# lilinitsy/skele-raytracer

Hardware: AMD Instinct MI355X
Metric: Mrays/sec + frame ms, 1920x1080 gillum=16 spheres2.scn (higher is better)
Workload: dtype f32

## Files before the change

skele_raytracer_amd/csrc/api.cpp:

```cpp
#include <hip/hip_runtime.h>

#include <cmath>
#include <cstdlib>
#include <cstdio>
#include <cstring>
#include <initializer_list>
#include <memory>
#include <vector>

#include "launch.h"
#include "scene_host.h"

static thread_local const char *g_variant = "none";

#define SKR_HIP(call)                                                                                      \
	do                                                                                                     \
	{                                                                                                      \
		hipError_t e_ = (call);                                                                            \
		if(e_ != hipSuccess)                                                                               \
		{                                                                                                  \
			skr_set_error("%s failed: %s (%s:%d)", #call, hipGetErrorString(e_), __FILE__, __LINE__);     \
			return SKR_ERR_HIP;                                                                            \
		}                                                                                                  \
	} while(0)
// ... 2 lines not shown
	int device = 0;
	skr_scene_info info{};
	int lds_limit = 0;
	int pow_steps = 11;
	float4 *d_blob = nullptr;
	size_t blob_bytes = 0;
	float4 *d_camec = nullptr;
	unsigned long long *d_counters = nullptr;
	unsigned long long *d_tri_work = nullptr;
	size_t off_amb = 0, off_kd = 0, off_ks = 0, off_lights = 0, off_tris = 0, off_chunks = 0, off_tri_mats = 0;
	size_t off_fog = 0;
	int n_fog = 0;
	size_t off_spot = 0;
	int n_spot = 0, spot_first = 0;
	size_t off_smask = 0;
	float shadow_reach2 = 0.0f;
	size_t off_gi = 0;
	SkrGiGrid gi_grid[2] = {};
	uint32_t gi_mask_word = 0;
	int gi_wide = 0;
	size_t gi_surface_word = 0;
	int n_chunks = 0, chunk_size = 0, cones = 0;
	size_t chunk_stride = 0;
	size_t off_trace = 0;
	float4 trace_ball{};
	int trace_cones = 0;
	bool tri_shadows = false;
	bool sphere_tree = false;
	size_t off_st_rows = 0, off_st_chunks = 0, off_st_nodes = 0;
	int st_nodes = 0, st_chunks = 0, st_always = 0;
// ... 63 lines not shown
	const int rc = r->nodes.grow(need);
	if(kept) *kept = rc == SKR_OK && was_kept && r->nodes.bytes == had;
	return rc;
}

static void load_switches(SkrSwitches &sw)
{
	sw = SkrSwitches();
	if(const char *e = getenv("SKR_PIPELINE"))
		sw.pipeline = !strcmp(e, "nodes") ? SKR_PIPE_NODES : !strcmp(e, "generic") ? SKR_PIPE_GENERIC : SKR_PIPE_OTHER;
	sw.no_cones = getenv("SKR_NO_CONES") != nullptr;
	sw.no_cull = getenv("SKR_NO_CULL") != nullptr;
	if(const char *e = getenv("SKR_NO_SPHERE_CULL")) sw.no_sphere_cull = atoi(e) > 0 ? 1 : 0;
	if(const char *e = getenv("SKR_LEVELS_BUDGET_MB")) sw.budget_mb = atoi(e) > 0 ? atoi(e) : 1;
	if(const char *e = getenv("SKR_FLAT")) sw.flat = atoi(e) > 0 ? 1 : -1;
	if(const char *e = getenv("SKR_SHADOW_MASK")) sw.shadow_mask = atoi(e) > 0 ? 1 : 0;
	if(const char *e = getenv("SKR_GI_MASK")) sw.gi_mask = atoi(e) > 0 ? 1 : 0;
	if(const char *e = getenv("SKR_GI_SURFACE")) sw.gi_surface = atoi(e) > 0 ? 1 : 0;
	if(const char *e = getenv("SKR_PRIMARY_CACHE")) sw.primary_cache = atoi(e) > 0 ? 1 : 0;
	if(const char *e = getenv("SKR_ADAPTIVE_PATH")) sw.adaptive_path = !strcmp(e, "frame") ? 1 : !strcmp(e, "query") ? 2 : 0;
}

void skr_copy_switches(skr_renderer *dst, const skr_renderer *src) { dst->sw = src->sw; }
int skr_render_tile_list_owned(skr_renderer *r, const skr_options *opt, uint32_t tile_rows, const uint32_t *d_tiles, uint32_t n_slots, uint64_t table_id, uint8_t *d_rgb,
							   float *d_rgbf, void *stream);

static std::vector<skr_f4> pack_scene(const skr_scene &s, DeviceScene &d)
{
	std::vector<skr_f4> rows;
	auto put = [&](const void *src, size_t bytes) {
		const size_t at = rows.size();
		rows.resize(at + (bytes + 15) / 16, skr_f4{0.0f, 0.0f, 0.0f, 0.0f});
		if(src && bytes) memcpy(&rows[at], src, bytes);
// ... 13 lines not shown
	d.n_chunks = s.info.n_triangles ? s.tri_node_count : 0;
	d.off_tri_mats = put4(s.tri_mats);
	d.off_fog = rows.size();
	d.n_fog = (int) (s.raw_fog.size() / 9);
	for(int j = 0; j < d.n_fog; j++)
	{
		const float *f = &s.raw_fog[9 * j];
		rows.push_back({f[3], f[8], f[7], 0.0f});
		rows.push_back({f[4], f[5], f[6], 0.0f});
	}
	d.n_spot = s.n_spot();
	d.spot_first = s.info.n_point_lights;
	d.off_spot = put4(s.spot_cones);
	if(!s.shadow_masks.empty()) d.off_smask = put(s.shadow_masks.data(), s.shadow_masks.size() * 4);
	d.shadow_reach2 = s.shadow_reach2;
	if(!s.gi_table.empty())
	{
		const size_t patch_word = s.gi_mask_word + (size_t) s.gi_rows * (SKR_GI_ROW_ENTRIES * (s.gi_wide ? 4 : 2) / 4);
		d.gi_surface_word = s.gi_surface.empty() ? 0 : patch_word + s.gi_surface_head;
		d.off_gi = put(nullptr, std::max(s.gi_table.size(), s.gi_surface.empty() ? 0 : patch_word + s.gi_surface.size()) * 4);
		uint32_t *words = reinterpret_cast<uint32_t *>(&rows[d.off_gi]);
		memcpy(words, s.gi_table.data(), s.gi_table.size() * 4);
		if(d.gi_surface_word) memcpy(words + patch_word, s.gi_surface.data(), s.gi_surface.size() * 4);
	}
	d.gi_grid[0] = s.gi_grid[0];
	d.gi_grid[1] = s.gi_grid[1];
	d.gi_mask_word = s.gi_mask_word;
	d.gi_wide = s.gi_wide;
	if(s.info.n_triangles && !s.trace_chunks.empty()) d.off_trace = put4(s.trace_chunks);
	d.trace_ball = make_float4(s.trace_ball[0], s.trace_ball[1], s.trace_ball[2], s.trace_ball[3]);
// ... 238 lines not shown
	const float *c = s.info.camera;
	p.background = f3{s.info.background[0], s.info.background[1], s.info.background[2]};
	p.n_spheres = s.info.n_spheres;
	p.n_tris = s.info.n_triangles;
	p.n_lights = s.info.n_point_lights + s.n_spot + s.info.n_directional_lights;
	p.sph_geom = s.d_blob;
	p.cam_ec = s.d_camec;
	p.sph_amb = s.d_blob + s.off_amb;
	p.sph_kd = s.d_blob + s.off_kd;
	p.sph_ks = s.d_blob + s.off_ks;
	p.lights = s.d_blob + s.off_lights;
	p.tris = s.d_blob + s.off_tris;
	p.tri_chunks = s.d_blob + s.off_chunks;
	p.tri_chunk_size = s.chunk_size;
	p.tri_cones = (s.cones && !r->sw.no_cones) ? 1 : 0;
	if(s.off_smask && r->sw.shadow_mask)
	{
		p.shadow_masks = reinterpret_cast<const uint32_t *>(s.d_blob + s.off_smask);
		p.shadow_reach2 = s.shadow_reach2;
		p.shadow_all = p.n_spheres >= 32 ? ~0u : (1u << p.n_spheres) - 1u;
	}
	if(s.off_gi && r->sw.gi_mask)
	{
		p.gi_index = reinterpret_cast<const int32_t *>(s.d_blob + s.off_gi);
		p.gi_masks = reinterpret_cast<const uint32_t *>(s.d_blob + s.off_gi) + s.gi_mask_word;
		p.gi_grid[0] = s.gi_grid[0];
		p.gi_grid[1] = s.gi_grid[1];
		p.gi_wide = s.gi_wide;
		p.gi_all = p.n_spheres >= 32 ? ~0u : (1u << p.n_spheres) - 1u;
		if(s.gi_surface_word && r->sw.gi_surface) p.gi_surface = reinterpret_cast<const uint32_t *>(s.d_blob + s.off_gi) + s.gi_surface_word;
	}
	{
		auto len3 = [](const float *v) { return std::sqrt((double) v[0] * v[0] + (double) v[1] * v[1] + (double) v[2] * v[2]); };
		const double umax = std::fabs((double) p.angle * p.aspect) * 1.001, vmax = std::fabs((double) p.angle) * 1.001;
		const double dmax = len3(c + 3) + umax * len3(c + 9) + vmax * len3(c + 6);
// ... 884 lines not shown
```

skele_raytracer_amd/csrc/render_params.h:

```cpp
#pragma once

#include <hip/hip_runtime.h>
#include <stdint.h>

#include "shadow_cells.h"

struct f3 {
	float x, y, z;
};

#define SKR_COUNTER_SHARDS 4096u
#ifndef SKR_PULL_QUEUES
#define SKR_PULL_QUEUES 16u
#endif
#define SKR_PULL_STRIDE 256u
#define SKR_P1_REGIONS 64u
#define SKR_PREFIX_WORDS (SKR_P1_REGIONS + 1u)

enum SkrPipeline { SKR_PIPE_AUTO = 0, SKR_PIPE_NODES, SKR_PIPE_GENERIC, SKR_PIPE_OTHER };
struct SkrSwitches {
	int32_t pipeline = SKR_PIPE_AUTO;
	int8_t no_cones = 0, no_cull = 0;
	int8_t primary_cache = 1;
	int8_t no_sphere_cull = 0;
	int32_t budget_mb = 0;
	int32_t flat = 0;
	int8_t shadow_mask = 1;
	int8_t gi_mask = 1;
	int8_t gi_surface = 1;
	int8_t adaptive_path = 0;
};

static_assert(sizeof(SkrSwitches) == 20, "SkrSwitches keeps its 20 bytes");

struct RenderParams {
	SkrSwitches sw;
	int32_t width, height;
	uint32_t tile_rows, first_tile, tile_stride, out_rows;
	const uint32_t *tile_table;
	uint32_t band_row0, band_rows;
	float inv_width, inv_height, aspect, angle;
	f3 cam_pos, cam_dir, cam_up, cam_right, background;
	int32_t n_spheres, n_tris, n_lights;
	const float4 *sph_geom, *sph_amb, *sph_kd, *sph_ks, *lights, *tris;
	const float4 *cam_ec;
	const float4 *tri_chunks;
	int32_t tri_chunk_size;
	int32_t tri_cones;
	int32_t n_tri_chunks;
	int32_t monte_carlo, num_path_traces, grid_size, max_depth, use_shadows;
	uint32_t seed_lo, seed_hi;
	int32_t pow_steps;
	uint8_t *rgb;
	float *rgbf;
	unsigned long long *counters;
	unsigned long long *tri_work;
	uint32_t *qctr;
	float *acc;
	uint32_t aa_index;
	uint32_t fog_row;
	const float4 *nd_src;
	const float4 *ns_src;
	float4 *nd_dst, *ns_dst;
	uint32_t nd_src_level0;
	const uint32_t *nd_count;
	float4 *rc;
	uint32_t rc_cap;
	uint32_t *rc_ctr;
	uint4 *ixh;
	uint32_t band_blk0, band_nblk, blocks_x;
	void *node_scratch;
	const float *res_in;
	float *res_out;
	int32_t shade_triangles;
	int32_t legacy_reflect;
	const float4 *tri_mats;
	uint32_t g_level;
	uint32_t g_arity;
	uint32_t g_last;
// ... 1 lines not shown
	const float4 *g_nodes_src;
	union {
		float4 *g_nodes_dst;
		int32_t *gi_row0;
	};
	const uint32_t *shadow_masks;
	float shadow_reach2;
	uint32_t shadow_all;
	const int32_t *gi_index;
	const uint32_t *gi_masks;
	SkrGiGrid gi_grid[2];
	int32_t gi_wide;
	uint32_t gi_all;
	const uint32_t *gi_surface;
};

struct SphereTree {
	const float4 *nodes;
	const float4 *chunks;
	const float4 *rows;
	int32_t n_nodes;
	int32_t n_chunks;
	int32_t n_always;
	int32_t cull;
	float4 ball;
	unsigned long long *work;
};

struct SpotLights {
	const float4 *cones;
// ... 21 lines not shown
```

skele_raytracer_amd/csrc/scene_host.cpp:

```cpp
#include "scene_host.h"

#include <cstdarg>
#include <cstdio>
#include <cstdlib>
#include <cstring>
#include <algorithm>
#include <cmath>
#include <fstream>

static thread_local char g_err[512] = "";

void skr_set_error(const char *fmt, ...)
{
	va_list ap;
	va_start(ap, fmt);
	vsnprintf(g_err, sizeof g_err, fmt, ap);
	va_end(ap);
}

extern "C" const char *skr_last_error(void) { return g_err; }

namespace {

int read_floats(const char *p, float *dst, int n)
// ... 79 lines not shown
	{
		const float *t = &raw_triangles[(size_t) order[i] * 9];
		tris[3 * i] = {t[0], t[1], t[2], 0.0f};
		float file_index;
		const int32_t fi = order[i];
		memcpy(&file_index, &fi, 4);
		tris[3 * i + 1] = {t[3] - t[0], t[4] - t[1], t[5] - t[2], file_index};
		tris[3 * i + 2] = {t[6] - t[0], t[7] - t[1], t[8] - t[2], 0.0f};
	}
	tri_order = order;
	build_triangle_materials();
	build_triangle_chunks();
	build_shadow_masks();
	build_gi_masks();
	build_gi_surface();
}

void skr_scene::build_lights()
{
	const int nl = info.n_point_lights, nsp = n_spot();
	const int nd = (int) (raw_directional_lights.size() / 6);
	lights.resize((size_t) (nl + nsp + nd) * 2);
	for(int i = 0; i < nl; i++)
	{
		const float *l = &raw_point_lights[(size_t) i * 6];
		lights[2 * i] = {l[0], l[1], l[2], 0.0f};
		lights[2 * i + 1] = {l[3], l[4], l[5], 0.0f};
	}
	spot_cones.resize((size_t) nsp * 2);
	for(int i = 0; i < nsp; i++)
// ... 126 lines not shown
			const double S = qn + rk;
			const double base = rk + eps_o + eta * (S + D + eps_o) / (1.0 - eta) + 0x1p-30 * qn;
			for(int c = 0; c < SKR_SHADOW_TABLE_WORDS; c++)
			{
				const double *wc = &cell_dir[3 * (size_t) c];
				const double s = q[0] * wc[0] + q[1] * wc[1] + q[2] * wc[2];
				const double dist = std::sqrt(std::max(0.0, qq - s * s));
				if(dist <= base + cell_theta[c] * S) masks[(size_t) l * SKR_SHADOW_TABLE_WORDS + c] |= 1u << k;
			}
		}
	}
	shadow_masks.swap(masks);
	shadow_reach2 = reach2;
}

static void gi_ball_bits(const double *q, double rho, const double *C, double r2, uint32_t bit, const std::vector<double> &cell_dir,
						 const std::vector<double> &cth, const std::vector<double> &sth, uint32_t *row)
{
	const double v[3] = {C[0] - q[0], C[1] - q[1], C[2] - q[2]};
	const double dist = std::sqrt(v[0] * v[0] + v[1] * v[1] + v[2] * v[2]);
	const double E = (dist + rho) * (1.0 + 0x1p-20);
	const double rk = std::sqrt(r2 + 0x1p-16 * (E * E + r2)) + 0x1p-20 * E;
	const double tol = 0x1p-30 * (dist + rho + rk);
	const double behind = rho + 0x1p-16 * E + tol;
	const double reach = rk + rho + tol;
	if(dist <= reach)
	{
		for(int e = 0; e < SKR_GI_ROW_ENTRIES; e++) row[e] |= bit;
		return;
	}
	for(int e = 0; e < SKR_GI_ROW_ENTRIES; e++)
	{
		const double *w = &cell_dir[3 * (size_t) e];
		const double cp = (v[0] * w[0] + v[1] * w[1] + v[2] * w[2]) / dist;
		const double x = v[1] * w[2] - v[2] * w[1], y = v[2] * w[0] - v[0] * w[2], z = v[0] * w[1] - v[1] * w[0];
		const double sp = std::sqrt(x * x + y * y + z * z) / dist;
		const double ct = cth[e], st = sth[e];
		const bool lo0 = cp >= ct;
		const bool hipi = cp <= -ct;
		const double cos_lo = lo0 ? 1.0 : cp * ct + sp * st;
		const double sin_lo = lo0 ? 0.0 : sp * ct - cp * st;
		const double sin_hi = hipi ? 0.0 : sp * ct + cp * st;
		const double min_sin = std::max(0.0, std::min(sin_lo, sin_hi));
		if(dist * cos_lo + behind >= 0.0 && dist * min_sin <= reach) row[e] |= bit;
	}
}

void skr_scene::build_gi_masks()
{
	gi_table.clear();
	gi_grid[0] = gi_grid[1] = SkrGiGrid{};
	gi_mask_word = 0;
	gi_wide = 0;
	const int ns = info.n_spheres;
	if(ns < 1 || ns > SKR_GI_MAX_SPHERES || info.n_triangles > 0) return;
	std::vector<double> C((size_t) 3 * ns), r2(ns), rad(ns);
	for(int k = 0; k < ns; k++)
	{
		C[3 * k] = sph_geom[k].x;
		C[3 * k + 1] = sph_geom[k].y;
// ... 107 lines not shown
	}
	std::vector<uint32_t> masks(cells.size() * SKR_GI_ROW_ENTRIES, 0u);
	for(size_t ci = 0; ci < cells.size(); ci++)
		for(int k = 0; k < ns; k++) gi_ball_bits(cells[ci].q, cells[ci].rho, &C[3 * k], r2[k], 1u << k, cell_dir, cth, sth, &masks[ci * SKR_GI_ROW_ENTRIES]);
	const size_t n_index = (index.size() + 1) & ~(size_t) 1;
	const size_t n_mask_words = gi_wide ? masks.size() : masks.size() / 2;
	std::vector<uint32_t> table((n_index + n_mask_words + 3) & ~(size_t) 3, 0u);
	memcpy(table.data(), index.data(), index.size() * 4);
	if(gi_wide) memcpy(&table[n_index], masks.data(), masks.size() * 4);
	else
		for(size_t e = 0; e < masks.size(); e += 2) table[n_index + e / 2] = masks[e] | masks[e + 1] << 16;
	gi_mask_word = (uint32_t) n_index;
	gi_table.swap(table);
}

void skr_scene::build_gi_surface()
{
	gi_surface.clear();
	gi_surface_head = 0;
	gi_rows = 0;
	if(gi_table.empty()) return;
	const int ns = info.n_spheres;
	const size_t row_words = (size_t) SKR_GI_ROW_ENTRIES * (gi_wide ? 4 : 2) / 4;
	gi_rows = (uint32_t) ((gi_table.size() - gi_mask_word) / row_words);
	std::vector<double> C((size_t) 3 * ns), r2(ns), rad(ns), R_lo(ns), R_hi(ns);
	std::vector<float> tau(ns);
	for(int k = 0; k < ns; k++)
	{
		C[3 * k] = sph_geom[k].x;
		C[3 * k + 1] = sph_geom[k].y;
		C[3 * k + 2] = sph_geom[k].z;
		r2[k] = sph_geom[k].w;
		rad[k] = std::sqrt(r2[k]);
		tau[k] = rad[k] > 1e-3 ? (float) (r2[k] * 0x1p-7) : -1.0f;
		R_lo[k] = std::sqrt(std::max(0.0, (r2[k] - tau[k]) * (1.0 - 0x1p-20))) * (1.0 - 0x1p-22);
		R_hi[k] = std::sqrt((r2[k] + std::max(0.0f, tau[k])) * (1.0 + 0x1p-20)) * (1.0 + 0x1p-22);
	}
	double blo[3], bhi[3];
	for(int c = 0; c < 3; c++)
	{
		blo[c] = gi_grid[0].lo[c];
		bhi[c] = blo[c] + gi_grid[0].n[c] / (double) gi_grid[0].inv;
	}
	struct Patch {
		int s, cell;
		double q[3], rho;
	};
	std::vector<Patch> patches;
	std::vector<int> G(ns, 0);
	std::vector<std::vector<double>> cdir(ns), cth(ns);
	size_t n_index = 0;
	bool fits = false;
	std::vector<double> sorted(rad);
	std::sort(sorted.begin(), sorted.end());
	double small_area = 0.0;
	for(int k = 0; k < ns; k++)
		if(rad[k] <= 4.0 * sorted[ns / 2]) small_area += 24.0 * r2[k];
	double edge = std::max(1e-6, 0.5 * std::sqrt(small_area / std::max(1.0, (double) SKR_GI_MAX_BYTES / (row_words * 4))));
	for(int attempt = 0; attempt < 200 && !fits; attempt++, edge *= 1.15)
	{
		patches.clear();
		n_index = 0;
		for(int k = 0; k < ns; k++)
		{
			const int g = tau[k] < 0.0f ? 0 : (int) std::min((double) SKR_GI_SURFACE_MAX_CELLS, std::max(1.0, std::ceil(2.0 * rad[k] / edge)));
			if(g != G[k])
			{
				G[k] = g;
				cdir[k].clear();
				cth[k].clear();
				if(g) cube_cells(g, cdir[k], cth[k]);
				for(double &t : cth[k]) t = t * (1.0 + 0x1p-20) + 0x1p-20;
			}
			n_index += (size_t) 6 * g * g;
			for(int cell = 0; cell < 6 * g * g; cell++)
			{
				const double *w = &cdir[k][3 * (size_t) cell];
				const double th = cth[k][cell], h = rad[k] * std::cos(th);
				Patch pt;
				pt.s = k;
				pt.cell = cell;
				for(int c = 0; c < 3; c++) pt.q[c] = C[3 * k + c] + h * w[c];
				double far = 0.0;
				for(double R : {R_lo[k], R_hi[k]}) far = std::max(far, std::sqrt(std::max(0.0, R * R + h * h - 2.0 * R * h * std::cos(th))));
				double cmax = 0.0;
				for(int c = 0; c < 3; c++) cmax = std::max(cmax, std::fabs(C[3 * k + c]));
				pt.rho = far * (1.0 + 0x1p-20) + 0x1p-30 * (cmax + rad[k]);
				double gap2 = 0.0;
				for(int c = 0; c < 3; c++)
				{
					const double o = std::max(0.0, std::max(blo[c] - pt.q[c], pt.q[c] - bhi[c]));
					gap2 += o * o;
				}
				if(gap2 <= pt.rho * pt.rho) patches.push_back(pt);
			}
		}
		fits = (SKR_GI_SURFACE_HEAD * (size_t) ns + n_index) * 4 + patches.size() * row_words * 4 <= SKR_GI_MAX_BYTES;
	}
	if(!fits || patches.empty()) return;
	std::vector<double> cell_dir, cell_theta;
	cube_cells(SKR_GI_DIR_CELLS, cell_dir, cell_theta);
	std::vector<double> dth(SKR_GI_ROW_ENTRIES), dct(SKR_GI_ROW_ENTRIES), dst(SKR_GI_ROW_ENTRIES);
	for(int e = 0; e < SKR_GI_ROW_ENTRIES; e++)
	{
		dth[e] = cell_theta[e] * (1.0 + 0x1p-20) + 0x1p-40;
		dct[e] = std::cos(dth[e]);
		dst[e] = std::sin(dth[e]);
	}
	std::vector<uint32_t> masks(patches.size() * SKR_GI_ROW_ENTRIES, 0u);
	for(size_t pi = 0; pi < patches.size(); pi++)
	{
		const Patch &pt = patches[pi];
		uint32_t *row = &masks[pi * SKR_GI_ROW_ENTRIES];
		for(int k = 0; k < ns; k++)
// ... 19 lines not shown
	int32_t *index = reinterpret_cast<int32_t *>(head + SKR_GI_SURFACE_HEAD * ns);
	size_t at = SKR_GI_SURFACE_HEAD * (size_t) ns;
	for(int k = 0; k < ns; k++)
	{
		head[SKR_GI_SURFACE_HEAD * k] = (uint32_t) at;
		head[SKR_GI_SURFACE_HEAD * k + 1] = (uint32_t) G[k];
		const float t = G[k] ? tau[k] : -1.0f;
		memcpy(&head[SKR_GI_SURFACE_HEAD * k + 2], &t, 4);
		for(int c = 0; c < 6 * G[k] * G[k]; c++) head[at + c] = 0xffffffffu;
		at += (size_t) 6 * G[k] * G[k];
	}
	for(size_t pi = 0; pi < patches.size(); pi++)
		index[head[SKR_GI_SURFACE_HEAD * patches[pi].s] - SKR_GI_SURFACE_HEAD * ns + patches[pi].cell] = (int32_t) (gi_rows + pi);
	gi_surface_head = (uint32_t) n_mask_words;
	gi_surface.swap(table);
}

void skr_scene::build_triangle_chunks()
{
	tri_chunks.clear();
	tri_any_cone = false;
	if(info.n_triangles == 0) return;
	const double dmax[SKR_CULL_LEVELS] = SKR_CULL_DMAX_LIST;
	for(int level = 0; level < SKR_CULL_LEVELS; level++)
	{
		std::vector<skr_f4> one;
		build_triangle_chunk_level(dmax[level], one);
		tri_chunk_stride = one.size();
		tri_chunks.insert(tri_chunks.end(), one.begin(), one.end());
	}
// ... 808 lines not shown
{
	if(!scene || n < 0 || n > SKR_SPOT_MAX_LIGHTS || (n && !rows))
	{
		skr_set_error("skr_scene_set_spot_lights: bad argument (at most %d spot lights)", SKR_SPOT_MAX_LIGHTS);
		return SKR_ERR_ARG;
	}
	for(int32_t i = 0; i < n; i++)
		if(!skr_spot_row_ok(rows + (size_t) i * 11))
		{
			skr_set_error("skr_scene_set_spot_lights: row %d is not a spot light (11 finite numbers, a direction other than zero, 0 <= angle1 <= angle2 <= 180)", i);
			return SKR_ERR_ARG;
		}
	scene->raw_spot_lights.assign(rows, rows + (size_t) n * 11);
	scene->build_lights();
	scene->build_shadow_masks();
	return SKR_OK;
}

int skr_scene_get_spot_lights(const skr_scene *scene, float *rows, int32_t *n)
{
	if(!scene) return SKR_ERR_ARG;
	if(n) *n = (int32_t) scene->n_spot();
	if(rows && !scene->raw_spot_lights.empty()) memcpy(rows, scene->raw_spot_lights.data(), scene->raw_spot_lights.size() * 4);
	return SKR_OK;
}

int skr_scene_get_spot_cones(const skr_scene *scene, float *cones)
{
	if(!scene) return SKR_ERR_ARG;
	for(int i = 0; cones && i < scene->n_spot(); i++)
// ... 162 lines not shown
			const SkrGiGrid &G = scene->gi_grid[g];
			const float row[8] = {G.lo[0], G.lo[1], G.lo[2], G.inv, (float) G.n[0], (float) G.n[1], (float) G.n[2], (float) G.base};
			memcpy(grids + 8 * g, row, sizeof(row));
		}
	if(table && !scene->gi_table.empty()) memcpy(table, scene->gi_table.data(), scene->gi_table.size() * 4);
	return SKR_OK;
}

int skr_scene_get_gi_surface(const skr_scene *scene, int32_t *n_words, int32_t *head_word, int32_t *first_row, uint32_t *table)
{
	if(!scene) return SKR_ERR_ARG;
	if(n_words) *n_words = (int32_t) scene->gi_surface.size();
	if(head_word) *head_word = (int32_t) scene->gi_surface_head;
	if(first_row) *first_row = (int32_t) scene->gi_rows;
	if(table && !scene->gi_surface.empty()) memcpy(table, scene->gi_surface.data(), scene->gi_surface.size() * 4);
	return SKR_OK;
}

void skr_options_default(skr_options *opt)
{
	if(!opt) return;
	opt->width = 1920;
	opt->height = 1080;
	opt->fov = 60;
	opt->monte_carlo = 0;
	opt->num_path_traces = 1;
	opt->grid_size = 0;
	opt->max_depth = 3;
	opt->use_shadows = 0;
	opt->seed = 1;
// ... 130 lines not shown
```

skele_raytracer_amd/csrc/scene_host.h:

```cpp
#pragma once

#include <cstdint>
#include <string>
#include <vector>

#include "../../include/skr.h"
#include "shadow_cells.h"
#include "tri_chunks.h"


struct skr_f4 {
	float x, y, z, w;
};

struct skr_scene {
	std::vector<float> raw_spheres;
	std::vector<float> raw_sphere_ior;
	std::vector<float> raw_triangles;
	std::vector<float> raw_triangle_materials;
	std::vector<float> raw_point_lights;
	std::vector<float> raw_directional_lights;
	std::vector<float> raw_fog;
	std::vector<float> raw_spot_lights;
	bool strict = false;
// ... 24 lines not shown
	void build_triangle_chunk_level(double d_max, std::vector<skr_f4> &out, const double *origin_ball = nullptr);
	std::vector<skr_f4> trace_chunks;
	float trace_ball[4] = {0.0f, 0.0f, 0.0f, 0.0f};
	bool trace_any_cone = false;
	std::vector<uint32_t> shadow_masks;
	float shadow_reach2 = 0.0f;
	void build_shadow_masks();
	std::vector<uint32_t> gi_table;
	SkrGiGrid gi_grid[2] = {};
	uint32_t gi_mask_word = 0;
	int gi_wide = 0;
	void build_gi_masks();
	std::vector<uint32_t> gi_surface;
	uint32_t gi_surface_head = 0;
	uint32_t gi_rows = 0;
	void build_gi_surface();
};

#define SKR_SPHERE_CHUNK 4
#define SKR_SPHERE_SUPER 8
struct SkrSphereTree {
	int n_nodes = 0, n_chunks = 0, n_always = 0;
	std::vector<skr_f4> rows;
	std::vector<int32_t> file;
	std::vector<skr_f4> nodes;
	std::vector<skr_f4> chunks;
	float ball[4] = {0.0f, 0.0f, 0.0f, -1.0f};
};
void skr_build_sphere_tree(const skr_scene &scene, SkrSphereTree &out);

bool skr_spot_row_ok(const float row[11]);
// ... 5 lines not shown
```

skele_raytracer_amd/csrc/shade_common.h:

```cpp
#pragma once

#include "device_math.h"
#include "render_params.h"
#include "shadow_cells.h"
#include "tri_chunks.h"

namespace {


struct SceneView {
	const float4 *geom;
	const float4 *amb;
	const float4 *kd;
	const float4 *ks;
	const float4 *lights;
	const float4 *tris;
	int ns, nt, nl;
	const float4 *chunks;
	int nchunks;
	int chunk;
	int cones;
	unsigned long long *tri_work;
	const float4 *geom_u;
	const uint32_t *smask;
// ... 355 lines not shown
	occ1 = !second;
	auto test = [&](const float4 g, int i) { pair_any_step(rp, pa, o, g, i, occ0, occ1, tests); };
	if(COHERENT) table_rows<SKR_COHERENT_TRIP>(sv.geom_u, sv.ns, test, [&] { return !__all(occ0 && occ1); });
	else if(sv.smask)
	{
		diag_mask_gate(19, cand, sv.ns);
		masked_rows(sv, cand, test);
	}
	else sphere_rows(sv, test);
	if(!occ0) tests += (uint32_t) sv.ns;
	if(second && !occ1) tests += (uint32_t) sv.ns;
	if(!second) occ1 = false;
}

template <bool COHERENT>
SKR_DEV uint32_t shadow_cands(const SceneView &sv, const RenderParams &p, int i, bool second, f3 P)
{
	if(COHERENT || !sv.smask || !p.use_shadows) return 0u;
	const uint32_t m0 = shadow_mask_of(sv, i, ld3(sv.lights[2 * i]) - P);
	return second ? m0 | shadow_mask_of(sv, i + 1, ld3(sv.lights[2 * i + 2]) - P) : m0;
}

SKR_DEV bool sphere_entry_touched(f3 o, f3 d, float dd, float4 A, float kappa)
{
	const f3 e = ld3(A) - o;
	const f3 cr = cross3(e, d);
	return !(dot3(cr, cr) > (A.w + kappa * dot3(e, e)) * dd);
}

SKR_DEV void sphere_work_add(const SphereTree &st, uint32_t n_cull, uint32_t n_sph)
{
	if(st.work && (n_cull | n_sph))
	{
// ... 193 lines not shown
	t.L = to_l * lt.inv;
	t.intensity = lt.inv2;
	return t;
}

struct NoTriangleShadows {
	static constexpr bool on = false;
};

struct SphereLoopShadows {
	static constexpr bool loops = true;
};

template <bool COHERENT, typename TS = NoTriangleShadows, typename SS = SphereLoopShadows>
SKR_DEV f3 direct_light_of(const SceneView &sv, const RenderParams &p, f3 kd, f3 ks, float4 ambp, f3 P, f3 N, Counters &cn, const TS &tri_shadows = TS(),
						   const SS &sphere_shadows = SS())
{
	f3 diffuse = mk3(0, 0, 0), specular = mk3(0, 0, 0);
	const f3 view = normalize3(p.cam_pos - P);
	for(int i = 0; i < sv.nl; i += 2)
	{
		const bool second = i + 1 < sv.nl;
		const uint32_t cand = SS::loops ? shadow_cands<COHERENT>(sv, p, i, second, P) : 0u;
		const LightTerm t0 = light_term(sv, i, P), t1 = light_term(sv, second ? i + 1 : i, P);
		bool occ0 = false, occ1 = false;
		if(p.use_shadows)
		{
			cn.shadow_rays += second ? 2u : 1u;
			if constexpr(SS::loops) occluded_pair<COHERENT>(sv, P, t0.L, t1.L, second, occ0, occ1, cn.shadow_tests, cand);
			else sphere_shadows.pair(sv, P, t0.L, t1.L, second, occ0, occ1, cn.shadow_tests);
			if constexpr(TS::on) tri_shadows(P, i, second, t0.L, t1.L, occ0, occ1);
		}
		auto add_light = [&](const LightTerm &t, bool lit)
		{
			if(lit)
			{
				diffuse = diffuse + ((kd * t.lc) * t.intensity) * max0(dot3(N, t.L));
				const f3 vl = view + t.L;
// ... 77 lines not shown
			}
		};
		add_light(t0, !occ0);
		add_light(t1, !occ1);
	}
	f3 total = mk3(0, 0, 0);
	total = total + ld3(ambp);
	total = total + diffuse;
	total = total + specular;
	return total;
}

template <bool COHERENT>
SKR_DEV f3 direct_light(const SceneView &sv, const RenderParams &p, int sph, f3 P, f3 N, Counters &cn)
{
	return direct_light_of<COHERENT>(sv, p, ld3(sv.kd[sph]), ld3(sv.ks[sph]), sv.amb[sph], P, N, cn);
}

SKR_DEV f3 fog_term(float4 a, float4 alb, const LightTerm &t, f3 centre, f3 lpos, f3 kd, f3 N, const uint32_t ctr[4], uint32_t k0, uint32_t k1,
					float *no_interaction_out = nullptr)
{
	float distance = length3(centre - lpos);
	if(distance > 2 * a.x) distance = 2 * a.x;
	const float no_interaction = (float) exp_spec((double) ((-1.0f * distance) * (a.y + a.z)));
	if(no_interaction_out) *no_interaction_out = no_interaction;
	uint32_t rnd[4];
	philox4x32(ctr[0], ctr[1], ctr[2], ctr[3], k0, k1, rnd);
	if(u31_to_unit(rnd[0]) > no_interaction) return ((kd * t.lc) * t.intensity) * max0(dot3(N, t.L));
	const f3 nd = mk3(t.L.x + u31_to_pm1(rnd[1]) * a.z, t.L.y + u31_to_pm1(rnd[2]) * a.z, t.L.z + u31_to_pm1(rnd[3]) * a.z);
	return (ld3(alb) * t.lc) * max0(dot3(N, nd));
}
// ... 335 lines not shown
```

skele_raytracer_amd/csrc/shadow_cells.h:

```cpp
#pragma once

#include <stdint.h>

#ifndef SKR_SHADOW_CELLS
#define SKR_SHADOW_CELLS 32
#endif
#define SKR_SHADOW_TABLE_WORDS (6 * SKR_SHADOW_CELLS * SKR_SHADOW_CELLS)
#define SKR_SHADOW_MAX_SPHERES 32

#ifndef SKR_GI_DIR_CELLS
#define SKR_GI_DIR_CELLS 16
#endif
#define SKR_GI_ROW_ENTRIES (6 * SKR_GI_DIR_CELLS * SKR_GI_DIR_CELLS)
#define SKR_GI_MAX_SPHERES 32
#define SKR_GI_MAX_BYTES (2u << 20)
struct SkrGiGrid {
	float lo[3], inv;
	float n_f[3];
	int32_t n[3], base;
};

#define SKR_GI_SURFACE_HEAD 4
#define SKR_GI_SURFACE_MAX_CELLS 128
```

Baseline: 62710.

## Add per-surface-patch precomputed shadow candidate masks for sphere hit points

Builds a host-side table that, for each light pair and each cube-mapped patch on every sphere's surface, conservatively lists which spheres could occlude the light. When a shading point lies on its sphere's surface, the kernel reads this tighter mask instead of the per-light direction-cell masks, so fewer sphere shadow tests run. It costs more scene-build time, up to 1 MB of extra table memory, and an extra head word packed into kd.w, and it relies on the conservative bounds being correct. It is enabled by default through the shadow_mask switch bit.

```diff
diff --git a/skele_raytracer_amd/csrc/api.cpp b/skele_raytracer_amd/csrc/api.cpp
--- a/skele_raytracer_amd/csrc/api.cpp
+++ b/skele_raytracer_amd/csrc/api.cpp
@@ -40,6 +40,8 @@
 	size_t off_spot = 0;
 	int n_spot = 0, spot_first = 0;
 	size_t off_smask = 0;
+	size_t off_ssurf = 0;
+	uint32_t ssurf_stride = 0;
 	float shadow_reach2 = 0.0f;
 	size_t off_gi = 0;
 	SkrGiGrid gi_grid[2] = {};
@@ -133,9 +135,10 @@
 	if(const char *e = getenv("SKR_NO_SPHERE_CULL")) sw.no_sphere_cull = atoi(e) > 0 ? 1 : 0;
 	if(const char *e = getenv("SKR_LEVELS_BUDGET_MB")) sw.budget_mb = atoi(e) > 0 ? atoi(e) : 1;
 	if(const char *e = getenv("SKR_FLAT")) sw.flat = atoi(e) > 0 ? 1 : -1;
-	if(const char *e = getenv("SKR_SHADOW_MASK")) sw.shadow_mask = atoi(e) > 0 ? 1 : 0;
+	if(const char *e = getenv("SKR_SHADOW_MASK")) sw.shadow_mask = (sw.shadow_mask & ~1) | (atoi(e) > 0 ? 1 : 0);
 	if(const char *e = getenv("SKR_GI_MASK")) sw.gi_mask = atoi(e) > 0 ? 1 : 0;
 	if(const char *e = getenv("SKR_GI_SURFACE")) sw.gi_surface = atoi(e) > 0 ? 1 : 0;
+	if(const char *e = getenv("SKR_SHADOW_SURFACE")) sw.shadow_mask = (sw.shadow_mask & ~2) | (atoi(e) > 0 ? 2 : 0);
 	if(const char *e = getenv("SKR_PRIMARY_CACHE")) sw.primary_cache = atoi(e) > 0 ? 1 : 0;
 	if(const char *e = getenv("SKR_ADAPTIVE_PATH")) sw.adaptive_path = !strcmp(e, "frame") ? 1 : !strcmp(e, "query") ? 2 : 0;
 }
@@ -179,6 +182,12 @@
 	d.off_spot = put4(s.spot_cones);
 	if(!s.shadow_masks.empty()) d.off_smask = put(s.shadow_masks.data(), s.shadow_masks.size() * 4);
 	d.shadow_reach2 = s.shadow_reach2;
+	if(!s.shadow_surface.empty())
+	{
+		d.off_ssurf = put(s.shadow_surface.data(), s.shadow_surface.size() * 4);
+		d.ssurf_stride = s.shadow_surface_stride;
+		for(size_t k = 0; k < s.shadow_surface_head.size(); k++) memcpy(&rows[d.off_kd + k].w, &s.shadow_surface_head[k], 4);
+	}
 	if(!s.gi_table.empty())
 	{
 		const size_t patch_word = s.gi_mask_word + (size_t) s.gi_rows * (SKR_GI_ROW_ENTRIES * (s.gi_wide ? 4 : 2) / 4);
@@ -447,11 +456,16 @@
 	p.tri_chunks = s.d_blob + s.off_chunks;
 	p.tri_chunk_size = s.chunk_size;
 	p.tri_cones = (s.cones && !r->sw.no_cones) ? 1 : 0;
-	if(s.off_smask && r->sw.shadow_mask)
+	if(s.off_smask && (r->sw.shadow_mask & 1))
 	{
 		p.shadow_masks = reinterpret_cast<const uint32_t *>(s.d_blob + s.off_smask);
 		p.shadow_reach2 = s.shadow_reach2;
 		p.shadow_all = p.n_spheres >= 32 ? ~0u : (1u << p.n_spheres) - 1u;
+		if(s.off_ssurf && (r->sw.shadow_mask & 2))
+		{
+			p.shadow_surface_word = (uint32_t) ((s.off_ssurf - s.off_smask) * 4);
+			p.shadow_surface_stride = s.ssurf_stride;
+		}
 	}
 	if(s.off_gi && r->sw.gi_mask)
 	{
diff --git a/skele_raytracer_amd/csrc/render_params.h b/skele_raytracer_amd/csrc/render_params.h
--- a/skele_raytracer_amd/csrc/render_params.h
+++ b/skele_raytracer_amd/csrc/render_params.h
@@ -25,7 +25,7 @@
 	int8_t no_sphere_cull = 0;
 	int32_t budget_mb = 0;
 	int32_t flat = 0;
-	int8_t shadow_mask = 1;
+	int8_t shadow_mask = 3;
 	int8_t gi_mask = 1;
 	int8_t gi_surface = 1;
 	int8_t adaptive_path = 0;
@@ -51,6 +51,7 @@
 	int32_t monte_carlo, num_path_traces, grid_size, max_depth, use_shadows;
 	uint32_t seed_lo, seed_hi;
 	int32_t pow_steps;
+	uint32_t shadow_surface_word;
 	uint8_t *rgb;
 	float *rgbf;
 	unsigned long long *counters;
@@ -63,6 +64,7 @@
 	const float4 *ns_src;
 	float4 *nd_dst, *ns_dst;
 	uint32_t nd_src_level0;
+	uint32_t shadow_surface_stride;
 	const uint32_t *nd_count;
 	float4 *rc;
 	uint32_t rc_cap;
@@ -94,6 +96,7 @@
 	uint32_t gi_all;
 	const uint32_t *gi_surface;
 };
+static_assert(sizeof(RenderParams) == 624, "RenderParams keeps its size: new fields go into its alignment holes");
 
 struct SphereTree {
 	const float4 *nodes;
diff --git a/skele_raytracer_amd/csrc/scene_host.cpp b/skele_raytracer_amd/csrc/scene_host.cpp
--- a/skele_raytracer_amd/csrc/scene_host.cpp
+++ b/skele_raytracer_amd/csrc/scene_host.cpp
@@ -117,6 +117,7 @@
 	build_shadow_masks();
 	build_gi_masks();
 	build_gi_surface();
+	build_shadow_surface();
 }
 
 void skr_scene::build_lights()
@@ -273,36 +274,53 @@
 	shadow_reach2 = reach2;
 }
 
+struct BallSphere {
+	double v[3], dist;
+	double rk;
+	double behind, reach;
+	bool meets;
+};
+static BallSphere ball_sphere(const double *q, double rho, const double *C, double r2)
+{
+	BallSphere b;
+	for(int c = 0; c < 3; c++) b.v[c] = C[c] - q[c];
+	b.dist = std::sqrt(b.v[0] * b.v[0] + b.v[1] * b.v[1] + b.v[2] * b.v[2]);
+	const double E = (b.dist + rho) * (1.0 + 0x1p-20);
+	b.rk = std::sqrt(r2 + 0x1p-16 * (E * E + r2)) + 0x1p-20 * E;
+	const double tol = 0x1p-30 * (b.dist + rho + b.rk);
+	b.behind = rho + 0x1p-16 * E + tol;
+	b.reach = b.rk + rho + tol;
+	b.meets = b.dist <= b.reach;
+	return b;
+}
+struct ConeSphere {
+	double cos_lo, min_sin;
+};
+static ConeSphere cone_sphere(const double *v, double dist, const double *w, double ct, double st)
+{
+	const double cp = (v[0] * w[0] + v[1] * w[1] + v[2] * w[2]) / dist;
+	const double x = v[1] * w[2] - v[2] * w[1], y = v[2] * w[0] - v[0] * w[2], z = v[0] * w[1] - v[1] * w[0];
+	const double sp = std::sqrt(x * x + y * y + z * z) / dist;
+	const bool lo0 = cp >= ct;
+	const bool hipi = cp <= -ct;
+	const double sin_lo = lo0 ? 0.0 : sp * ct - cp * st;
+	const double sin_hi = hipi ? 0.0 : sp * ct + cp * st;
+	return ConeSphere{lo0 ? 1.0 : cp * ct + sp * st, std::max(0.0, std::min(sin_lo, sin_hi))};
+}
+static bool cone_ahead(const ConeSphere &c, double dist, double behind) { return dist * c.cos_lo + behind >= 0.0; }
+static bool cone_line_touches(const ConeSphere &c, double dist, double reach) { return dist * c.min_sin <= reach; }
+static bool ball_cone_touches(const BallSphere &b, const double *w, double ct, double st)
+{
+	if(b.meets) return true;
+	const ConeSphere c = cone_sphere(b.v, b.dist, w, ct, st);
+	return cone_ahead(c, b.dist, b.behind) && cone_line_touches(c, b.dist, b.reach);
+}
 static void gi_ball_bits(const double *q, double rho, const double *C, double r2, uint32_t bit, const std::vector<double> &cell_dir,
 						 const std::vector<double> &cth, const std::vector<double> &sth, uint32_t *row)
 {
-	const double v[3] = {C[0] - q[0], C[1] - q[1], C[2] - q[2]};
-	const double dist = std::sqrt(v[0] * v[0] + v[1] * v[1] + v[2] * v[2]);
-	const double E = (dist + rho) * (1.0 + 0x1p-20);
-	const double rk = std::sqrt(r2 + 0x1p-16 * (E * E + r2)) + 0x1p-20 * E;
-	const double tol = 0x1p-30 * (dist + rho + rk);
-	const double behind = rho + 0x1p-16 * E + tol;
-	const double reach = rk + rho + tol;
-	if(dist <= reach)
-	{
-		for(int e = 0; e < SKR_GI_ROW_ENTRIES; e++) row[e] |= bit;
-		return;
-	}
+	const BallSphere b = ball_sphere(q, rho, C, r2);
 	for(int e = 0; e < SKR_GI_ROW_ENTRIES; e++)
-	{
-		const double *w = &cell_dir[3 * (size_t) e];
-		const double cp = (v[0] * w[0] + v[1] * w[1] + v[2] * w[2]) / dist;
-		const double x = v[1] * w[2] - v[2] * w[1], y = v[2] * w[0] - v[0] * w[2], z = v[0] * w[1] - v[1] * w[0];
-		const double sp = std::sqrt(x * x + y * y + z * z) / dist;
-		const double ct = cth[e], st = sth[e];
-		const bool lo0 = cp >= ct;
-		const bool hipi = cp <= -ct;
-		const double cos_lo = lo0 ? 1.0 : cp * ct + sp * st;
-		const double sin_lo = lo0 ? 0.0 : sp * ct - cp * st;
-		const double sin_hi = hipi ? 0.0 : sp * ct + cp * st;
-		const double min_sin = std::max(0.0, std::min(sin_lo, sin_hi));
-		if(dist * cos_lo + behind >= 0.0 && dist * min_sin <= reach) row[e] |= bit;
-	}
+		if(ball_cone_touches(b, &cell_dir[3 * (size_t) e], cth[e], sth[e])) row[e] |= bit;
 }
 
 void skr_scene::build_gi_masks()
@@ -440,17 +458,59 @@
 	gi_table.swap(table);
 }
 
+struct SurfaceShell {
+	float tau;
+	double R_lo, R_hi;
+};
+static SurfaceShell surface_shell(double r2)
+{
+	SurfaceShell sh;
+	sh.tau = std::sqrt(r2) > 1e-3 ? (float) (r2 * 0x1p-7) : -1.0f;
+	sh.R_lo = std::sqrt(std::max(0.0, (r2 - sh.tau) * (1.0 - 0x1p-20))) * (1.0 - 0x1p-22);
+	sh.R_hi = std::sqrt((r2 + std::max(0.0f, sh.tau)) * (1.0 + 0x1p-20)) * (1.0 + 0x1p-22);
+	return sh;
+}
+static void surface_patch_ball(const double *C, double rad, const SurfaceShell &sh, const double *w, double th, double *q, double &rho)
+{
+	const double h = rad * std::cos(th);
+	for(int c = 0; c < 3; c++) q[c] = C[c] + h * w[c];
+	double far = 0.0;
+	for(double R : {sh.R_lo, sh.R_hi}) far = std::max(far, std::sqrt(std::max(0.0, R * R + h * h - 2.0 * R * h * std::cos(th))));
+	double cmax = 0.0;
+	for(int c = 0; c < 3; c++) cmax = std::max(cmax, std::fabs(C[c]));
+	rho = far * (1.0 + 0x1p-20) + 0x1p-30 * (cmax + rad);
+}
+static void surface_cells(int g, std::vector<double> &dir, std::vector<double> &theta)
+{
+	dir.clear();
+	theta.clear();
+	if(g) cube_cells(g, dir, theta);
+	for(double &t : theta) t = t * (1.0 + 0x1p-20) + 0x1p-20;
+}
+static double surface_first_edge(const std::vector<double> &rad, const std::vector<double> &r2, double rows)
+{
+	const int ns = (int) rad.size();
+	std::vector<double> sorted(rad);
+	std::sort(sorted.begin(), sorted.end());
+	double small_area = 0.0;
+	for(int k = 0; k < ns; k++)
+		if(rad[k] <= 4.0 * sorted[ns / 2]) small_area += 24.0 * r2[k];
+	return std::max(1e-6, 0.5 * std::sqrt(small_area / std::max(1.0, rows)));
+}
+
 void skr_scene::build_gi_surface()
 {
 	gi_surface.clear();
 	gi_surface_head = 0;
 	gi_rows = 0;
+	gi_surface_edge = 0.0;
 	if(gi_table.empty()) return;
 	const int ns = info.n_spheres;
 	const size_t row_words = (size_t) SKR_GI_ROW_ENTRIES * (gi_wide ? 4 : 2) / 4;
 	gi_rows = (uint32_t) ((gi_table.size() - gi_mask_word) / row_words);
 	std::vector<double> C((size_t) 3 * ns), r2(ns), rad(ns), R_lo(ns), R_hi(ns);
 	std::vector<float> tau(ns);
+	std::vector<SurfaceShell> shell(ns);
 	for(int k = 0; k < ns; k++)
 	{
 		C[3 * k] = sph_geom[k].x;
@@ -458,9 +518,10 @@
 		C[3 * k + 2] = sph_geom[k].z;
 		r2[k] = sph_geom[k].w;
 		rad[k] = std::sqrt(r2[k]);
-		tau[k] = rad[k] > 1e-3 ? (float) (r2[k] * 0x1p-7) : -1.0f;
-		R_lo[k] = std::sqrt(std::max(0.0, (r2[k] - tau[k]) * (1.0 - 0x1p-20))) * (1.0 - 0x1p-22);
-		R_hi[k] = std::sqrt((r2[k] + std::max(0.0f, tau[k])) * (1.0 + 0x1p-20)) * (1.0 + 0x1p-22);
+		shell[k] = surface_shell(r2[k]);
+		tau[k] = shell[k].tau;
+		R_lo[k] = shell[k].R_lo;
+		R_hi[k] = shell[k].R_hi;
 	}
 	double blo[3], bhi[3];
 	for(int c = 0; c < 3; c++)
@@ -477,12 +538,7 @@
 	std::vector<std::vector<double>> cdir(ns), cth(ns);
 	size_t n_index = 0;
 	bool fits = false;
-	std::vector<double> sorted(rad);
-	std::sort(sorted.begin(), sorted.end());
-	double small_area = 0.0;
-	for(int k = 0; k < ns; k++)
-		if(rad[k] <= 4.0 * sorted[ns / 2]) small_area += 24.0 * r2[k];
-	double edge = std::max(1e-6, 0.5 * std::sqrt(small_area / std::max(1.0, (double) SKR_GI_MAX_BYTES / (row_words * 4))));
+	double edge = surface_first_edge(rad, r2, (double) SKR_GI_MAX_BYTES / (row_words * 4)), used_edge = 0.0;
 	for(int attempt = 0; attempt < 200 && !fits; attempt++, edge *= 1.15)
 	{
 		patches.clear();
@@ -493,25 +549,15 @@
 			if(g != G[k])
 			{
 				G[k] = g;
-				cdir[k].clear();
-				cth[k].clear();
-				if(g) cube_cells(g, cdir[k], cth[k]);
-				for(double &t : cth[k]) t = t * (1.0 + 0x1p-20) + 0x1p-20;
+				surface_cells(g, cdir[k], cth[k]);
 			}
 			n_index += (size_t) 6 * g * g;
 			for(int cell = 0; cell < 6 * g * g; cell++)
 			{
-				const double *w = &cdir[k][3 * (size_t) cell];
-				const double th = cth[k][cell], h = rad[k] * std::cos(th);
 				Patch pt;
 				pt.s = k;
 				pt.cell = cell;
-				for(int c = 0; c < 3; c++) pt.q[c] = C[3 * k + c] + h * w[c];
-				double far = 0.0;
-				for(double R : {R_lo[k], R_hi[k]}) far = std::max(far, std::sqrt(std::max(0.0, R * R + h * h - 2.0 * R * h * std::cos(th))));
-				double cmax = 0.0;
-				for(int c = 0; c < 3; c++) cmax = std::max(cmax, std::fabs(C[3 * k + c]));
-				pt.rho = far * (1.0 + 0x1p-20) + 0x1p-30 * (cmax + rad[k]);
+				surface_patch_ball(&C[3 * k], rad[k], shell[k], &cdir[k][3 * (size_t) cell], cth[k][cell], pt.q, pt.rho);
 				double gap2 = 0.0;
 				for(int c = 0; c < 3; c++)
 				{
@@ -522,8 +568,10 @@
 			}
 		}
 		fits = (SKR_GI_SURFACE_HEAD * (size_t) ns + n_index) * 4 + patches.size() * row_words * 4 <= SKR_GI_MAX_BYTES;
+		if(fits) used_edge = edge;
 	}
 	if(!fits || patches.empty()) return;
+	gi_surface_edge = used_edge;
 	std::vector<double> cell_dir, cell_theta;
 	cube_cells(SKR_GI_DIR_CELLS, cell_dir, cell_theta);
 	std::vector<double> dth(SKR_GI_ROW_ENTRIES), dct(SKR_GI_ROW_ENTRIES), dst(SKR_GI_ROW_ENTRIES);
@@ -573,6 +621,107 @@
 		index[head[SKR_GI_SURFACE_HEAD * patches[pi].s] - SKR_GI_SURFACE_HEAD * ns + patches[pi].cell] = (int32_t) (gi_rows + pi);
 	gi_surface_head = (uint32_t) n_mask_words;
 	gi_surface.swap(table);
+}
+
+void skr_scene::build_shadow_surface(double rho_scale, double cone_scale)
+{
+	shadow_surface.clear();
+	shadow_surface_head.clear();
+	shadow_surface_stride = 0;
+	if(shadow_masks.empty()) return;
+	const int ns = info.n_spheres, nl = (int) (shadow_masks.size() / SKR_SHADOW_TABLE_WORDS), npairs = (nl + 1) / 2;
+	std::vector<double> C((size_t) 3 * ns), r2(ns), rad(ns);
+	std::vector<SurfaceShell> shell(ns);
+	for(int k = 0; k < ns; k++)
+	{
+		C[3 * k] = sph_geom[k].x;
+		C[3 * k + 1] = sph_geom[k].y;
+		C[3 * k + 2] = sph_geom[k].z;
+		r2[k] = sph_geom[k].w;
+		rad[k] = std::sqrt(r2[k]);
+		for(int c = 0; c < 3; c++)
+			if(!(std::fabs(C[3 * k + c]) < 1e6)) return;
+		if(!(rad[k] < 1e6)) return;
+		shell[k] = surface_shell(r2[k]);
+	}
+	double edge = gi_surface_edge > 0.0 ? gi_surface_edge : surface_first_edge(rad, r2, (double) SKR_GI_MAX_BYTES / (SKR_GI_ROW_ENTRIES * (ns > 16 ? 4 : 2)));
+	edge /= SKR_SHADOW_SURFACE_SCALE;
+	std::vector<int> G(ns, 0);
+	size_t stride = 0;
+	for(int attempt = 0; attempt < 200; attempt++, edge *= 1.15)
+	{
+		stride = 0;
+		for(int k = 0; k < ns; k++)
+		{
+			G[k] = shell[k].tau < 0.0f ? 0 : (int) std::min((double) SKR_GI_SURFACE_MAX_CELLS, std::max(1.0, std::ceil(2.0 * rad[k] / edge)));
+			stride += (size_t) 6 * G[k] * G[k];
+		}
+		if(stride * npairs * 4 <= SKR_SHADOW_SURFACE_MAX_BYTES) break;
+	}
+	if(stride == 0 || stride * npairs * 4 > SKR_SHADOW_SURFACE_MAX_BYTES) return;
+	const uint32_t all = ns >= 32 ? 0xffffffffu : (1u << ns) - 1u;
+	const double eta = 0x1p-15;
+	std::vector<uint32_t> table(stride * npairs, 0u), head(ns, 0u);
+	std::vector<double> cdir, cth;
+	std::vector<BallSphere> bs(ns);
+	size_t base = 0;
+	for(int s = 0; s < ns; s++)
+	{
+		head[s] = (uint32_t) base | (uint32_t) G[s] << 24;
+		surface_cells(G[s], cdir, cth);
+		double cmax = 0.0;
+		for(int c = 0; c < 3; c++) cmax = std::max(cmax, std::fabs(C[3 * s + c]));
+		const double eps_o = 2.0 * std::sqrt(3.0) * (1e-6 + 0x1p-23 * (cmax + shell[s].R_hi + 1e-6));
+		const double R_in = shell[s].R_lo - eps_o;
+		const double E_own = (shell[s].R_hi + eps_o) * (1.0 + 0x1p-20);
+		const double behind_own = 0x1p-16 * E_own + 0x1p-30 * shell[s].R_hi;
+		const double tilt = R_in > 0.0 ? std::asin(std::min(1.0, eps_o / shell[s].R_lo)) : 0.0;
+		for(int cell = 0; cell < 6 * G[s] * G[s]; cell++)
+		{
+			const double *wp = &cdir[3 * (size_t) cell];
+			double q[3], rho;
+			surface_patch_ball(&C[3 * s], rad[s], shell[s], wp, cth[cell], q, rho);
+			rho = (rho + eps_o) * rho_scale;
+			for(int k = 0; k < ns; k++)
+				if(k != s) bs[k] = ball_sphere(q, rho, &C[3 * k], r2[k]);
+			for(int l = 0; l < nl; l++)
+			{
+				uint32_t &word = table[(size_t) (l >> 1) * stride + base + cell];
+				const skr_f4 &lp = lights[2 * (size_t) l];
+				const double d[3] = {lp.x - q[0], lp.y - q[1], lp.z - q[2]};
+				const double dl = std::sqrt(d[0] * d[0] + d[1] * d[1] + d[2] * d[2]);
+				if(!(dl > rho * (1.0 + 0x1p-20) + 0x1p-30 * (cmax + rad[s])))
+				{
+					word = all;
+					continue;
+				}
+				const double w[3] = {d[0] / dl, d[1] / dl, d[2] / dl};
+				const double theta = (std::asin(std::min(1.0, rho / dl)) * (1.0 + 0x1p-20) + eta) * cone_scale;
+				const double ct = std::cos(theta), st = std::sin(theta);
+				const double near_l = eps_o + eta * (dl + rho) * (1.0 + 0x1p-20);
+				const double lpd[3] = {lp.x, lp.y, lp.z};
+				for(int k = 0; k < ns; k++)
+				{
+					if(k == s) continue;
+					const BallSphere &b = bs[k];
+					const bool ahead = b.meets || cone_ahead(cone_sphere(b.v, b.dist, w, ct, st), b.dist, b.behind);
+					const double vl[3] = {C[3 * k] - lpd[0], C[3 * k + 1] - lpd[1], C[3 * k + 2] - lpd[2]};
+					const double distl = std::sqrt(vl[0] * vl[0] + vl[1] * vl[1] + vl[2] * vl[2]);
+					const double reach_l = b.rk + near_l + 0x1p-30 * (distl + dl + b.rk);
+					const bool line = distl <= reach_l || cone_line_touches(cone_sphere(vl, distl, w, ct, st), distl, reach_l);
+					if(ahead && line) word |= 1u << k;
+				}
+				const double x = wp[1] * w[2] - wp[2] * w[1], y = wp[2] * w[0] - wp[0] * w[2], z = wp[0] * w[1] - wp[1] * w[0];
+				const double psi = std::atan2(std::sqrt(x * x + y * y + z * z), wp[0] * w[0] + wp[1] * w[1] + wp[2] * w[2]);
+				const double ang = psi + cth[cell] + tilt + theta + 0x1p-30;
+				if(!(R_in > 0.0 && ang < 0.5 * M_PI && R_in * std::cos(ang) > behind_own)) word |= 1u << s;
+			}
+		}
+		base += (size_t) 6 * G[s] * G[s];
+	}
+	shadow_surface_stride = (uint32_t) stride;
+	shadow_surface.swap(table);
+	shadow_surface_head.swap(head);
 }
 
 void skr_scene::build_triangle_chunks()
@@ -1411,6 +1560,7 @@
 	scene->raw_spot_lights.assign(rows, rows + (size_t) n * 11);
 	scene->build_lights();
 	scene->build_shadow_masks();
+	scene->build_shadow_surface();
 	return SKR_OK;
 }
 
@@ -1603,6 +1753,23 @@
 	if(head_word) *head_word = (int32_t) scene->gi_surface_head;
 	if(first_row) *first_row = (int32_t) scene->gi_rows;
 	if(table && !scene->gi_surface.empty()) memcpy(table, scene->gi_surface.data(), scene->gi_surface.size() * 4);
+	return SKR_OK;
+}
+
+int skr_scene_get_shadow_surface(const skr_scene *scene, int32_t *n_pairs, int32_t *stride, uint32_t *head, uint32_t *table)
+{
+	if(!scene) return SKR_ERR_ARG;
+	if(stride) *stride = (int32_t) scene->shadow_surface_stride;
+	if(n_pairs) *n_pairs = scene->shadow_surface_stride ? (int32_t) (scene->shadow_surface.size() / scene->shadow_surface_stride) : 0;
+	if(head && !scene->shadow_surface_head.empty()) memcpy(head, scene->shadow_surface_head.data(), scene->shadow_surface_head.size() * 4);
+	if(table && !scene->shadow_surface.empty()) memcpy(table, scene->shadow_surface.data(), scene->shadow_surface.size() * 4);
+	return SKR_OK;
+}
+
+int skr_scene_rebuild_shadow_surface(skr_scene *scene, double rho_scale, double cone_scale)
+{
+	if(!scene) return SKR_ERR_ARG;
+	scene->build_shadow_surface(rho_scale, cone_scale);
 	return SKR_OK;
 }
 
diff --git a/skele_raytracer_amd/csrc/scene_host.h b/skele_raytracer_amd/csrc/scene_host.h
--- a/skele_raytracer_amd/csrc/scene_host.h
+++ b/skele_raytracer_amd/csrc/scene_host.h
@@ -62,7 +62,11 @@
 	std::vector<uint32_t> gi_surface;
 	uint32_t gi_surface_head = 0;
 	uint32_t gi_rows = 0;
+	double gi_surface_edge = 0.0;
 	void build_gi_surface();
+	std::vector<uint32_t> shadow_surface, shadow_surface_head;
+	uint32_t shadow_surface_stride = 0;
+	void build_shadow_surface(double rho_scale = 1.0, double cone_scale = 1.0);
 };
 
 #define SKR_SPHERE_CHUNK 4
diff --git a/skele_raytracer_amd/csrc/shade_common.h b/skele_raytracer_amd/csrc/shade_common.h
--- a/skele_raytracer_amd/csrc/shade_common.h
+++ b/skele_raytracer_amd/csrc/shade_common.h
@@ -393,9 +393,21 @@
 }
 
 template <bool COHERENT>
-SKR_DEV uint32_t shadow_cands(const SceneView &sv, const RenderParams &p, int i, bool second, f3 P)
+SKR_DEV uint32_t shadow_cands(const SceneView &sv, const RenderParams &p, int i, bool second, f3 P, int sph = -1)
 {
 	if(COHERENT || !sv.smask || !p.use_shadows) return 0u;
+	if(p.shadow_surface_word != 0u && (uint32_t) sph < (uint32_t) sv.ns)
+	{
+		const float4 g = sv.geom[sph];
+		const uint32_t head = __float_as_uint(sv.kd[sph].w), n = head >> 24;
+		const f3 e = P - ld3(g);
+		const float c = dot3(e, e) - g.w;
+		if(n != 0u && __builtin_fabsf(c) <= g.w * SKR_SURFACE_SLACK)
+		{
+			const CubeCell cc = cube_cell_n(e, (int) n);
+			return sv.smask[p.shadow_surface_word + (uint32_t) (i >> 1) * p.shadow_surface_stride + (head & 0xffffffu) + ((uint32_t) cc.face * n + (uint32_t) cc.i) * n + (uint32_t) cc.j];
+		}
+	}
 	const uint32_t m0 = shadow_mask_of(sv, i, ld3(sv.lights[2 * i]) - P);
 	return second ? m0 | shadow_mask_of(sv, i + 1, ld3(sv.lights[2 * i + 2]) - P) : m0;
 }
@@ -619,14 +631,14 @@
 
 template <bool COHERENT, typename TS = NoTriangleShadows, typename SS = SphereLoopShadows>
 SKR_DEV f3 direct_light_of(const SceneView &sv, const RenderParams &p, f3 kd, f3 ks, float4 ambp, f3 P, f3 N, Counters &cn, const TS &tri_shadows = TS(),
-						   const SS &sphere_shadows = SS())
+						   const SS &sphere_shadows = SS(), int sph = -1)
 {
 	f3 diffuse = mk3(0, 0, 0), specular = mk3(0, 0, 0);
 	const f3 view = normalize3(p.cam_pos - P);
 	for(int i = 0; i < sv.nl; i += 2)
 	{
 		const bool second = i + 1 < sv.nl;
-		const uint32_t cand = SS::loops ? shadow_cands<COHERENT>(sv, p, i, second, P) : 0u;
+		const uint32_t cand = SS::loops ? shadow_cands<COHERENT>(sv, p, i, second, P, sph) : 0u;
 		const LightTerm t0 = light_term(sv, i, P), t1 = light_term(sv, second ? i + 1 : i, P);
 		bool occ0 = false, occ1 = false;
 		if(p.use_shadows)
@@ -734,7 +746,7 @@
 template <bool COHERENT>
 SKR_DEV f3 direct_light(const SceneView &sv, const RenderParams &p, int sph, f3 P, f3 N, Counters &cn)
 {
-	return direct_light_of<COHERENT>(sv, p, ld3(sv.kd[sph]), ld3(sv.ks[sph]), sv.amb[sph], P, N, cn);
+	return direct_light_of<COHERENT>(sv, p, ld3(sv.kd[sph]), ld3(sv.ks[sph]), sv.amb[sph], P, N, cn, NoTriangleShadows(), SphereLoopShadows(), sph);
 }
 
 SKR_DEV f3 fog_term(float4 a, float4 alb, const LightTerm &t, f3 centre, f3 lpos, f3 kd, f3 N, const uint32_t ctr[4], uint32_t k0, uint32_t k1,
diff --git a/skele_raytracer_amd/csrc/shadow_cells.h b/skele_raytracer_amd/csrc/shadow_cells.h
--- a/skele_raytracer_amd/csrc/shadow_cells.h
+++ b/skele_raytracer_amd/csrc/shadow_cells.h
@@ -7,6 +7,12 @@
 #endif
 #define SKR_SHADOW_TABLE_WORDS (6 * SKR_SHADOW_CELLS * SKR_SHADOW_CELLS)
 #define SKR_SHADOW_MAX_SPHERES 32
+
+#define SKR_SURFACE_SLACK 0x1p-7f
+#ifndef SKR_SHADOW_SURFACE_SCALE
+#define SKR_SHADOW_SURFACE_SCALE 4
+#endif
+#define SKR_SHADOW_SURFACE_MAX_BYTES (1u << 20)
 
 #ifndef SKR_GI_DIR_CELLS
 #define SKR_GI_DIR_CELLS 16
```

New measurement: 64330, median of 6. +2.6%, better.
